# xkuubix/MonteCarlo-Gated-MIL

Measured on AMD Instinct MI355X. Metric: bags/sec × MCDO-samples (T=100) at N=2048,d=512; 1/2/4/8-GPU + %HBM roofline, higher is better.
Workload: dtype bf16

## Files before the change

montecarlo-gated-mil_amd/csrc/mcgmil_kernels.h:

```cpp
#pragma once
#include "mcgmil_device.h"

namespace mcgmil {

struct GateParams {
    const void* H;
    long long ldh;
    const int32_t* bag_off;
    int B, T, L, D, C, G, P;
    long long total_samples;
    const void* Wp;
    uint32_t wp_bytes;
    const float* bv;
    const float* bu;
    const float* wa;
    const float* ba;
    float sf, sa;
    uint32_t thr_f, thr_a;
    uint32_t thrx_f;
    uint32_t k0, k1;
    uint32_t bag_base;
    int t_base;
    const uint32_t* bag_ids;
    const int32_t* tile_bag;
// ... 59 lines not shown
            bag = (int)(R / per_bag);
            const long long local = R - (long long)bag * per_bag;
            t = (int)(local / Nb);
            n = (int)(local - (long long)t * Nb);
        }
        hrow = bag * Nb + n;
    } else if (R < p.total_samples) {
        if (p.tile_bag) {
            bag = p.tile_bag[R0 / BM];
            while ((long long)p.T * p.bag_off[bag + 1] <= R) ++bag;
        } else {
            bag = find_bag(p.bag_off, p.B, p.T, R);
        }
        const int ob = p.bag_off[bag];
        Nb = p.bag_off[bag + 1] - ob;
        const long long local = R - (long long)p.T * ob;
        if (narrow) {
            t = (int)((uint32_t)local / (uint32_t)Nb);
            n = (int)((uint32_t)local - (uint32_t)t * (uint32_t)Nb);
        } else {
            t = (int)(local / Nb);
            n = (int)(local - (long long)t * Nb);
        }
        hrow = ob + n;
    }
    int* ri = rinfo + kRowInfo * tid;
    ri[0] = hrow; ri[1] = t; ri[2] = n; ri[3] = bag; ri[4] = Nb;
    ri[5] = (int)(p.bag_ids ? p.bag_ids[bag] : p.bag_base + (uint32_t)bag);
}

#ifndef MCGMIL_KERNELS_TEMPLATES_ONLY
__global__ void plan_tiles_kernel(const int32_t* bag_off, int B, int T, long long total_samples,
                                  int BM, long long tiles, int32_t* tile_bag) {
    const long long i = (long long)blockIdx.x * blockDim.x + threadIdx.x;
    if (i >= tiles) return;
    const long long R = i * BM;
    tile_bag[i] = R < total_samples ? find_bag(bag_off, B, T, R) : 0;
}
#endif

__device__ __forceinline__ float gated_product_scaled(float ax, float by) {
    ax = fminf(fmaxf(ax, -43.280851226668903f), 43.280851226668903f);
    const float a = __builtin_amdgcn_exp2f(ax);
    const float b = __builtin_amdgcn_exp2f(by);
    const float ia = 1.0f + a;
    return (1.0f - a) * __builtin_amdgcn_rcpf(fmaf(ia, b, ia));
}

#ifndef MCGMIL_DIAG
#define MCGMIL_DIAG 0
#endif
#ifndef MCGMIL_PHILOX_ROUNDS
#define MCGMIL_PHILOX_ROUNDS 10
#endif

constexpr float kM2Log2e = -2.8853900817779268f;
constexpr float kMLog2e = -1.4426950408889634f;

struct HeadVec { f32x4 bv, bu, wa; };

template <int PPW>
__device__ __forceinline__ void load_head_vectors(const GateParams& p, int q0, int lane,
                                                  HeadVec (&hv)[PPW]) {
    const int DB = p.D >> 4;
#pragma unroll
    for (int jp = 0; jp < PPW; ++jp) {
        const int q = q0 + jp < p.P ? q0 + jp : p.P - 1;
        const int g = q / DB, db = q - g * DB;
        const int d0 = db * 16 + 4 * (lane >> 4);
        hv[jp].bv = *reinterpret_cast<const f32x4*>(p.bv + (size_t)g * p.D + d0) * kM2Log2e;
        hv[jp].bu = *reinterpret_cast<const f32x4*>(p.bu + (size_t)g * p.D + d0) * kMLog2e;
        hv[jp].wa = *reinterpret_cast<const f32x4*>(p.wa + (size_t)g * p.D + d0);
    }
}

struct Region {
    int bag, t0, t1, Nb, ob;
    int ntiles;
    long long S, rows;
};

constexpr int kFusedTiles = 32;
constexpr int kFusedHv = 256;
struct alignas(16) FusedConst {
    Region rg;
    uint32_t bagctr;
    int pad0;
    float ba[4];
    int cls[8];
    int pad1[8];
    int4 tile[kFusedTiles];
    float hv[3][kFusedHv];
};

#ifndef MCGMIL_FUSED_HV_LDS
#define MCGMIL_FUSED_HV_LDS 1
#endif
template <int PPW>
__device__ __forceinline__ void load_head_vectors_lds(const FusedConst* fc, int P, int q0, int lane,
                                                      HeadVec (&hv)[PPW]) {
#pragma unroll
    for (int jp = 0; jp < PPW; ++jp) {
        const int q = q0 + jp < P ? q0 + jp : P - 1;
        const int d = 16 * q + 4 * (lane >> 4);
        hv[jp].bv = *reinterpret_cast<const f32x4*>(fc->hv[0] + d);
        hv[jp].bu = *reinterpret_cast<const f32x4*>(fc->hv[1] + d);
        hv[jp].wa = *reinterpret_cast<const f32x4*>(fc->hv[2] + d);
    }
}

template <int RT, int PPW, int MAXC, bool ONE_CLASS, int RTV = RT>
__device__ __forceinline__ void fold_pairs(const GateParams& p, const f32x4 (&acc)[RT][2 * PPW],
                                           int q0, int lane, float (&part)[MAXC][RT],
                                           const HeadVec* pre = nullptr) {
    const int DB = p.D >> 4;
    const float av_s = p.sf * kM2Log2e, au_s = p.sf * kMLog2e;
#pragma unroll
    for (int jp = 0; jp < PPW; ++jp) {
        const int q = q0 + jp;
        if (q >= p.P) break;
        const int col = 16 * q + 4 * (lane >> 4);
        const int g = ONE_CLASS ? 0 : q / DB;
        const int d0 = col - g * p.D;
        f32x4 bvv, buv;
        f32x4 coef[MAXC];
        if (ONE_CLASS && pre) {
            bvv = pre[jp].bv;
            buv = pre[jp].bu;
            coef[0] = pre[jp].wa;
#pragma unroll
            for (int c = 1; c < MAXC; ++c) coef[c] = f32x4{0.f, 0.f, 0.f, 0.f};
        } else {
            bvv = *reinterpret_cast<const f32x4*>(p.bv + col);
            buv = *reinterpret_cast<const f32x4*>(p.bu + col);
            bvv *= kM2Log2e;
            buv *= kMLog2e;
#pragma unroll
            for (int c = 0; c < MAXC; ++c) {
                const int cc = ONE_CLASS ? g : c;
                const bool use = ONE_CLASS ? (c == 0) : ((c < p.C) && (p.G == 1 || c == g));
                const f32x4 w = *reinterpret_cast<const f32x4*>(p.wa + (size_t)(use ? cc : 0) * p.D + d0);
                coef[c] = use ? w : f32x4{0.f, 0.f, 0.f, 0.f};
            }
        }
#pragma unroll
        for (int rt = 0; rt < RTV; ++rt) {
#pragma unroll
            for (int v = 0; v < 4; ++v) {
                const float ax = fmaf(acc[rt][2 * jp][v], av_s, bvv[v]);
                const float by = fmaf(acc[rt][2 * jp + 1][v], au_s, buv[v]);
                if constexpr (ONE_CLASS) {
#if MCGMIL_DIAG & 8
                    part[0][rt] = fmaf(fmaf(ax, coef[0][v], by), ax, part[0][rt]);
                    continue;
#endif
                    const float a = __builtin_amdgcn_exp2f(fminf(fmaxf(ax, -43.280851226668903f),
                                                                 43.280851226668903f));
                    const float b = __builtin_amdgcn_exp2f(by);
                    const float ia = 1.0f + a;
                    const float r = __builtin_amdgcn_rcpf(fmaf(ia, b, ia));
                    part[0][rt] = fmaf(fmaf(-a, coef[0][v], coef[0][v]), r, part[0][rt]);
                } else {
                    const float pr = gated_product_scaled(ax, by);
#pragma unroll
                    for (int c = 0; c < MAXC; ++c) part[c][rt] = fmaf(pr, coef[c][v], part[c][rt]);
                }
            }
        }
    }
}

template <int BM, int MAXC>
__host__ __device__ constexpr int red_floats() { return kGateWaves * MAXC * 4 * BM; }

template <int BM, int MAXC, int ROWS = 16, bool AFFINE = false>
__device__ __forceinline__ void finish_scores(const GateParams& p, long long R0,
                                              float (&part)[MAXC][BM / ROWS], f32x4 zacc,
                                              bool zwave, float* red, float* zred,
                                              const int* rinfo, int one_class, int waves_per_gate,
                                              bool have_keep, bool keep, float* lg_out,
                                              float* z_out, long long obase,
                                              const FusedConst* fc = nullptr, int tile = 0) {
    constexpr int RT = BM / ROWS;
    constexpr int NG = 64 / ROWS;
    const int tid = threadIdx.x, lane = tid & 63, wave = tid >> 6;
    const int ncls = one_class < 0 ? MAXC : 1;
#pragma unroll
    for (int c = 0; c < MAXC; ++c) {
        if (c >= ncls) break;
        const int cls = one_class < 0 ? c : one_class;
        if (cls >= MAXC) break;
        float* dst = red + ((size_t)(wave * MAXC + cls) * NG + lane / ROWS) * BM + (lane % ROWS);
#pragma unroll
        for (int q = 0; q < RT; ++q) dst[ROWS * q] = part[c][q];
    }
    if (zwave && lane < 16) {
#pragma unroll
        for (int c = 0; c < MAXC; ++c) zred[c * BM + wave * 16 + lane] = zacc[c];
    }
    MCGMIL_STAMP(p, 5);
    __syncthreads();
    MCGMIL_STAMP(p, 6);
    const int r = wave * 16 + (lane & 15), c = lane >> 4;
    if (r >= BM || c >= p.C) return;
    int t, n, bag, Nb;
    uint32_t bagc;
    size_t orow;
    float bias;
    if constexpr (AFFINE) {
        const int4 tl = fc->tile[tile];
        t = tl.x, n = tl.y + r, bag = fc->rg.bag, Nb = fc->rg.Nb;
        bagc = fc->bagctr;
        orow = (size_t)(tl.z + r);
        bias = fc->ba[c];
    } else {
        const int* ri = rinfo + kRowInfo * r;
        if (ri[0] < 0) return;
        t = ri[1], n = ri[2], bag = ri[3], Nb = ri[4];
        bagc = (uint32_t)ri[5];
        orow = (size_t)(R0 + r - obase);
        bias = p.ba[c];
    }
    float s = 0.f;
    const int nw = waves_per_gate ? waves_per_gate : kGateWaves;
    for (int k = 0; k < nw; ++k) {
        const int w = waves_per_gate ? c * waves_per_gate + k : k;
        const float* src = red + (size_t)(w * MAXC + c) * NG * BM + r;
#pragma unroll
        for (int g = 0; g < NG; ++g) s += src[g * BM];
    }
    s += bias;
    if (p.keep_att) {
        const size_t abase = (size_t)p.T * p.C * (size_t)p.bag_off[bag];
        keep = p.keep_att[abase + ((size_t)t * p.C + c) * Nb + n] != 0;
    } else if (!have_keep) {
        keep = attention_keep(p.k0, p.k1, bagc, (uint32_t)(p.t_base + t), (uint32_t)c,
                              (uint32_t)n, p.thr_a);
    }
    const size_t o = orow * p.C + c;
    lg_out[o] = s * (keep ? p.sa : 0.f);
    z_out[o] = zred[c * BM + r] * p.sf;
}

constexpr int kSoftmaxRows = 16;

#ifndef MCGMIL_NT_A
#define MCGMIL_NT_A 1
#endif
__device__ __forceinline__ void store_a(float* dst, float v) {
#if MCGMIL_NT_A
    __builtin_nontemporal_store(v, dst);
#else
    *dst = v;
#endif
}

__device__ __forceinline__ void softmax_group(int ltid, bool active, int Nb, int C, const float* lg,
                                              const float* zz, float* Ao, float* Yo, float* sred) {
    const int tid = ltid, lane = ltid & 63, wave = ltid >> 6;
    if (Nb == 0) {
        if (active && tid < C) Yo[tid] = 0.f;
        return;
    }
    const int Nl = active ? Nb : 0;
    if (C == 2 && Nb <= 256 * kSoftmaxRows) {
        float (*sred2)[4] = reinterpret_cast<float (*)[4]>(sred);
        float e0[kSoftmaxRows], e1[kSoftmaxRows];
        float2 zr[kSoftmaxRows];
        float m0 = -INFINITY, m1 = -INFINITY;
#pragma unroll
        for (int k = 0; k < kSoftmaxRows; ++k) {
            const int n = tid + 256 * k;
            float2 l = make_float2(-INFINITY, -INFINITY);
            zr[k] = make_float2(0.f, 0.f);
            if (n < Nl) {
                l = *reinterpret_cast<const float2*>(lg + (size_t)n * 2);
                zr[k] = *reinterpret_cast<const float2*>(zz + (size_t)n * 2);
            }
            e0[k] = l.x;
            e1[k] = l.y;
            m0 = fmaxf(m0, e0[k]);
            m1 = fmaxf(m1, e1[k]);
        }
        m0 = wave_max(m0);
        m1 = wave_max(m1);
        if (lane == 0) { sred2[0][wave] = m0; sred2[1][wave] = m1; }
        __syncthreads();
        m0 = fmaxf(fmaxf(sred2[0][0], sred2[0][1]), fmaxf(sred2[0][2], sred2[0][3]));
        m1 = fmaxf(fmaxf(sred2[1][0], sred2[1][1]), fmaxf(sred2[1][2], sred2[1][3]));
        __syncthreads();
        float s0 = 0.f, y0 = 0.f, s1 = 0.f, y1 = 0.f;
#pragma unroll
        for (int k = 0; k < kSoftmaxRows; ++k) {
            const int n = tid + 256 * k;
            if (n < Nl) {
                const float2 z = zr[k];
                e0[k] = expf(e0[k] - m0);
                e1[k] = expf(e1[k] - m1);
                s0 += e0[k];
                s1 += e1[k];
                y0 = fmaf(e0[k], z.x, y0);
                y1 = fmaf(e1[k], z.y, y1);
            }
        }
        s0 = wave_sum(s0);
        y0 = wave_sum(y0);
        s1 = wave_sum(s1);
        y1 = wave_sum(y1);
        if (lane == 0) {
            sred2[0][wave] = s0; sred2[1][wave] = y0; sred2[2][wave] = s1; sred2[3][wave] = y1;
        }
        __syncthreads();
        s0 = (sred2[0][0] + sred2[0][1]) + (sred2[0][2] + sred2[0][3]);
        y0 = (sred2[1][0] + sred2[1][1]) + (sred2[1][2] + sred2[1][3]);
        s1 = (sred2[2][0] + sred2[2][1]) + (sred2[2][2] + sred2[2][3]);
        y1 = (sred2[3][0] + sred2[3][1]) + (sred2[3][2] + sred2[3][3]);
        __syncthreads();
// ... 52 lines not shown
                for (int k = 0; k < kSoftmaxRows; ++k) {
                    const int n = tid + 256 * k;
                    if (n < Nl) store_a(Aoc + n, e[k] * inv);
                }
            }
            if (active && tid == 0) Yo[c] = y * inv;
            continue;
        }
        float m = -INFINITY;
        for (int n = tid; n < Nl; n += 256) m = fmaxf(m, lg[(size_t)n * C + c]);
        m = wave_max(m);
        if (lane == 0) sr[0][wave] = m;
        __syncthreads();
        m = fmaxf(fmaxf(sr[0][0], sr[0][1]), fmaxf(sr[0][2], sr[0][3]));
        __syncthreads();
        float s = 0.f, y = 0.f;
        for (int n = tid; n < Nl; n += 256) {
            const size_t o = (size_t)n * C + c;
            const float e = expf(lg[o] - m);
            s += e;
            y = fmaf(e, zz[o], y);
        }
        s = wave_sum(s);
        y = wave_sum(y);
        if (lane == 0) { sr[0][wave] = s; sr[1][wave] = y; }
        __syncthreads();
        s = (sr[0][0] + sr[0][1]) + (sr[0][2] + sr[0][3]);
        y = (sr[1][0] + sr[1][1]) + (sr[1][2] + sr[1][3]);
        __syncthreads();
        const float inv = 1.0f / s;
        if (Ao) {
            float* Aoc = Ao + (size_t)c * Nb;
            for (int n = tid; n < Nl; n += 256) store_a(Aoc + n, expf(lg[(size_t)n * C + c] - m) * inv);
        }
        if (active && tid == 0) Yo[c] = y * inv;
    }
}

#ifndef MCGMIL_KERNELS_TEMPLATES_ONLY
__global__ __launch_bounds__(256) void softmax_pool_kernel(const int32_t* bag_off, int T, int C,
                                                           const float* logits, const float* zz,
                                                           float* Y, float* A) {
    __shared__ float sred[16];
    const int t = blockIdx.x, b = blockIdx.y;
    const int ob = bag_off[b];
    const int Nb = bag_off[b + 1] - ob;
    const size_t R0 = (size_t)T * ob + (size_t)t * Nb;
    softmax_group(threadIdx.x, true, Nb, C, logits + R0 * C, zz + R0 * C,
                  A ? A + (size_t)T * C * ob + (size_t)t * C * Nb : nullptr,
                  Y + ((size_t)b * T + t) * C, sred);
}
#endif

template <typename E> struct Raw;
template <> struct Raw<__bf16> { uint4 v; };
template <> struct Raw<float> { f32x4 lo, hi; };
__device__ __forceinline__ Raw<__bf16> load_raw(const __bf16* p) {
    Raw<__bf16> r; r.v = *reinterpret_cast<const uint4*>(p); return r;
}
__device__ __forceinline__ Raw<float> load_raw(const float* p) {
    Raw<float> r;
    r.lo = *reinterpret_cast<const f32x4*>(p);
    r.hi = *reinterpret_cast<const f32x4*>(p + 4);
    return r;
}
__device__ __forceinline__ void store_masked(const Raw<__bf16>& h, uint32_t kb, __bf16* dst) {
    uint4 v = h.v;
    v.x &= ((kb & 1u) ? 0x0000FFFFu : 0u) | ((kb & 2u) ? 0xFFFF0000u : 0u);
    v.y &= ((kb & 4u) ? 0x0000FFFFu : 0u) | ((kb & 8u) ? 0xFFFF0000u : 0u);
    v.z &= ((kb & 16u) ? 0x0000FFFFu : 0u) | ((kb & 32u) ? 0xFFFF0000u : 0u);
    v.w &= ((kb & 64u) ? 0x0000FFFFu : 0u) | ((kb & 128u) ? 0xFFFF0000u : 0u);
    *reinterpret_cast<uint4*>(dst) = v;
}
__device__ __forceinline__ void store_masked(const Raw<float>& h, uint32_t kb, float* dst) {
    f32x4 a = h.lo, b = h.hi;
    a.x = (kb & 1u) ? a.x : 0.f;   a.y = (kb & 2u) ? a.y : 0.f;
    a.z = (kb & 4u) ? a.z : 0.f;   a.w = (kb & 8u) ? a.w : 0.f;
    b.x = (kb & 16u) ? b.x : 0.f;  b.y = (kb & 32u) ? b.y : 0.f;
    b.z = (kb & 64u) ? b.z : 0.f;  b.w = (kb & 128u) ? b.w : 0.f;
    *reinterpret_cast<f32x4*>(dst) = a;
    *reinterpret_cast<f32x4*>(dst + 4) = b;
}

__device__ __forceinline__ void store_dropped(const Raw<__bf16>& h, uint4 o, uint32_t thrx,
                                              uint32_t inval, __bf16* dst) {
    uint4 v = h.v;
    v.x = __builtin_amdgcn_bitop3_b32(v.x, drop_mask16x2_flipped(o.x, thrx), inval, 0x10);
    v.y = __builtin_amdgcn_bitop3_b32(v.y, drop_mask16x2(o.y, thrx), inval, 0x10);
    v.z = __builtin_amdgcn_bitop3_b32(v.z, drop_mask16x2_flipped(o.z, thrx), inval, 0x10);
    v.w = __builtin_amdgcn_bitop3_b32(v.w, drop_mask16x2(o.w, thrx), inval, 0x10);
    *reinterpret_cast<uint4*>(dst) = v;
}
__device__ __forceinline__ uint32_t keep_lo(uint32_t m) { return ~(uint32_t)((int32_t)(m << 16) >> 16); }
__device__ __forceinline__ uint32_t keep_hi(uint32_t m) { return ~(uint32_t)((int32_t)m >> 16); }
__device__ __forceinline__ void store_dropped(const Raw<float>& h, uint4 o, uint32_t thrx,
                                              uint32_t inval, float* dst) {
    const uint32_t m0 = drop_mask16x2_flipped(o.x, thrx) | inval, m1 = drop_mask16x2(o.y, thrx) | inval;
    const uint32_t m2 = drop_mask16x2_flipped(o.z, thrx) | inval, m3 = drop_mask16x2(o.w, thrx) | inval;
    f32x4 a = h.lo, b = h.hi;
    a.x = __uint_as_float(__float_as_uint(a.x) & keep_lo(m0));
    a.y = __uint_as_float(__float_as_uint(a.y) & keep_hi(m0));
    a.z = __uint_as_float(__float_as_uint(a.z) & keep_lo(m1));
    a.w = __uint_as_float(__float_as_uint(a.w) & keep_hi(m1));
    b.x = __uint_as_float(__float_as_uint(b.x) & keep_lo(m2));
    b.y = __uint_as_float(__float_as_uint(b.y) & keep_hi(m2));
    b.z = __uint_as_float(__float_as_uint(b.z) & keep_lo(m3));
    b.w = __uint_as_float(__float_as_uint(b.w) & keep_hi(m3));
    *reinterpret_cast<f32x4*>(dst) = a;
    *reinterpret_cast<f32x4*>(dst + 4) = b;
}

constexpr int kPipeBM = 128;
#ifndef MCGMIL_VPM
#define MCGMIL_VPM 2
#endif
constexpr int VPM = MCGMIL_VPM;
#ifndef MCGMIL_SCHED
#define MCGMIL_SCHED 0
#endif
constexpr int HD = 2;
template <typename E>
__host__ __device__ constexpr int pipe_slots() { return 2; }

template <typename E, int MAXC>
__host__ __device__ constexpr size_t pipe_lds_bytes() {
    return (size_t)pipe_slots<E>() * kPipeBM * 32 * sizeof(E) + (size_t)red_floats<kPipeBM, MAXC>() * 4 +
           (size_t)MAXC * kPipeBM * 4 + (size_t)kRowInfo * kPipeBM * 4;
}

template <typename E>
__device__ __forceinline__ void load_classifier_lds(__amdgpu_buffer_rsrc_t wrs, uint32_t zsoff, int KS, E* zw) {
    for (int i = threadIdx.x; i < KS * 64; i += kGateThreads)
        *reinterpret_cast<f32x4*>(zw + (size_t)i * 8) = __builtin_bit_cast(
            f32x4, __builtin_amdgcn_raw_buffer_load_b128(wrs, (uint32_t)i * 8u * (uint32_t)sizeof(E), zsoff, 0));
}

template <typename E, int PPW, int MAXC, bool REPLAY, bool ONE_CLASS, bool EARLY_HV = true,
          bool ZL = false, bool ZLOAD = true, int RTV = kPipeBM / 16, bool AFFINE = false>
__device__ __forceinline__ void pipe_tile(const GateParams& p, long long R0, E* Xs, float* red,
                                          float* zred, const int* rinfo, float* lg_out,
                                          float* z_out, long long obase, E* zw = nullptr,
                                          const FusedConst* fc = nullptr, int tile = 0) {
    constexpr int BM = kPipeBM;
    constexpr int RT = BM / 16;
    constexpr int NJ = 2 * PPW;
    constexpr int SLOT = RT * 64 * 8;
    const int tid = threadIdx.x, lane = tid & 63, wave = tid >> 6;
    const int KS = p.L >> 5;

    int hrow;
    uint32_t cn, ct, cb;
    if constexpr (AFFINE) {
        static_assert(!REPLAY, "the affine rows have no replay masks");
        const int4 tl = fc->tile[tile];
        cn = (uint32_t)(tl.y + wave * 16 + (lane & 15));
        hrow = fc->rg.ob + (int)cn;
        ct = (uint32_t)(p.t_base + tl.x);
        cb = fc->bagctr;
    } else {
        const int* ri = rinfo + kRowInfo * (wave * 16 + (lane & 15));
        hrow = ri[0];
        cn = (uint32_t)ri[2], ct = (uint32_t)(p.t_base + ri[1]), cb = (uint32_t)ri[5];
    }
    const bool valid = AFFINE || hrow >= 0;
    const int kq = lane >> 4;
    const E* hsrc = reinterpret_cast<const E*>(p.H) + (size_t)(valid ? hrow : 0) * p.ldh + kq * 8;
    const uint8_t* kfe = REPLAY ? p.keep_feat + (size_t)(valid ? R0 + wave * 16 + (lane & 15) : 0) *
                                                    (p.L >> 3) + kq
                                : nullptr;

    const uint32_t inval = valid ? 0u : 0xFFFFFFFFu;
    auto stage = [&](int s, const Raw<E>& h, E* slot) {
        if constexpr (REPLAY) {
            const uint32_t kb = kfe[(size_t)(s < KS ? s : KS - 1) * 4];
            store_masked(h, kb & ~inval, slot + tid * 8);
        } else {
#if MCGMIL_DIAG & 4
            const uint4 o = make_uint4(cn * 0x9E3779B9u + (uint32_t)s, ct ^ cb, cn + ct, (uint32_t)s * 77u);
#else
            const uint4 o = philox4x32_10<true, MCGMIL_PHILOX_ROUNDS>((uint32_t)(s * 4 + kq), cn, ct, cb, p.k0, p.k1);
#endif
            store_dropped(h, o, p.thrx_f, inval, slot + tid * 8);
        }
    };

    const __amdgpu_buffer_rsrc_t wrs = make_rsrc(p.Wp, p.wp_bytes);
    const uint32_t tile_bytes = (uint32_t)KS * 512u * (uint32_t)sizeof(E);
    constexpr uint32_t kStepBytes = 512u * (uint32_t)sizeof(E);
    const int q0 = __builtin_amdgcn_readfirstlane(wave) * PPW;
    uint32_t wsoff[NJ];
#pragma unroll
    for (int j = 0; j < NJ; ++j) {
        int q = q0 + (j >> 1);
        q = q < p.P ? q : p.P - 1;
        wsoff[j] = (uint32_t)(2 * q + (j & 1)) * tile_bytes;
    }
    const uint32_t zsoff = (uint32_t)(2 * p.P) * tile_bytes;
    const uint32_t lane_b = (uint32_t)lane * 8u * (uint32_t)sizeof(E);
    auto wfrag = [&](uint32_t soff) { return load_frag_buf<E>(wrs, lane_b, soff); };

    f32x4 acc[RT][NJ];
#pragma unroll
    for (int rt = 0; rt < RT; ++rt)
#pragma unroll
        for (int j = 0; j < NJ; ++j) acc[rt][j] = f32x4{0.f, 0.f, 0.f, 0.f};
    f32x4 zacc = {0.f, 0.f, 0.f, 0.f};

    auto kstep = [&](int s, const E* cur, E* nxt, const Frag<E> (&w)[NJ], const Frag<E>& z,
                     Frag<E> (&wn)[NJ], Frag<E>& zn, const Raw<E>& h, Raw<E>& hn) {
        const int s1 = s + 1 < KS ? s + 1 : KS - 1;
        const int sh = s + HD < KS ? s + HD : KS - 1;
#if MCGMIL_DIAG & 2
#pragma unroll
        for (int j = 0; j < NJ; ++j) wn[j] = w[j];
        zn = z;
#else
#pragma unroll
        for (int j = 0; j < NJ; ++j) wn[j] = wfrag(wsoff[j] + (uint32_t)s1 * kStepBytes);
        if constexpr (!ZL) zn = wfrag(zsoff + (uint32_t)s1 * kStepBytes);
#endif
#if MCGMIL_DIAG & 1
        hn = h;
#else
        if (RTV == RT || wave < RTV) hn = load_raw(hsrc + (size_t)sh * 32);
#endif
#pragma unroll
        for (int rt = 0; rt < RTV; ++rt) {
            const Frag<E> x = load_frag(cur + (size_t)(rt * 64 + lane) * 8);
#pragma unroll
            for (int j = 0; j < NJ; ++j) acc[rt][j] = mma(w[j], x, acc[rt][j]);
        }
        const Frag<E> xz = load_frag(cur + (size_t)tid * 8);
        if constexpr (ZL) zacc = mma(load_frag(zw + (size_t)(s * 64 + lane) * 8), xz, zacc);
        else zacc = mma(z, xz, zacc);
        if (RTV == RT || wave < RTV) stage(s + 1, h, nxt);
        if constexpr (sizeof(E) == 2 && PPW == 2) {
#if MCGMIL_SCHED == 1
            __builtin_amdgcn_sched_group_barrier(0x020, NJ + 2, 0);
            __builtin_amdgcn_sched_group_barrier(0x100, 3, 0);
#pragma unroll
            for (int rt = 0; rt < RT; ++rt) {
#pragma unroll
                for (int j = 0; j < NJ; ++j) {
                    __builtin_amdgcn_sched_group_barrier(0x008, 1, 0);
                    __builtin_amdgcn_sched_group_barrier(0x002, VPM, 0);
                }
                if (rt + 2 < RT) __builtin_amdgcn_sched_group_barrier(0x100, 1, 0);
            }
            __builtin_amdgcn_sched_group_barrier(0x008, 1, 0);
            __builtin_amdgcn_sched_group_barrier(0x002, VPM, 0);
#else
#pragma unroll
            for (int i = 0; i < RTV * NJ + 1; ++i) {
                __builtin_amdgcn_sched_group_barrier(0x008, 1, 0);
                __builtin_amdgcn_sched_group_barrier(0x002, VPM, 0);
            }
#endif
        }
#if MCGMIL_DIAG & 128
        asm volatile("s_waitcnt lgkmcnt(0)" ::: "memory");
#else
        __syncthreads();
#endif
    };

    constexpr bool kEarlyHV = EARLY_HV && ONE_CLASS && sizeof(E) == 2;
    HeadVec hvec[PPW];
    {
        Frag<E> wA[NJ], wB[NJ], zA, zB;
        Raw<E> hA{}, hB{};
        if (RTV == RT || wave < RTV) {
            hA = load_raw(hsrc);
            hB = load_raw(hsrc + 32);
        }
#pragma unroll
        for (int j = 0; j < NJ; ++j) wA[j] = wfrag(wsoff[j]);
        if constexpr (ZL) {
            if constexpr (ZLOAD) load_classifier_lds<E>(wrs, zsoff, KS, zw);
        } else {
            zA = wfrag(zsoff);
        }
        if (RTV == RT || wave < RTV) stage(0, hA, Xs);
        __syncthreads();
        MCGMIL_STAMP(p, 2);

        if constexpr (kEarlyHV) load_head_vectors<PPW>(p, q0, lane, hvec);
        kstep(0, Xs, Xs + SLOT, wA, zA, wB, zB, hB, hA);
        kstep(1, Xs + SLOT, Xs, wB, zB, wA, zA, hA, hB);
#if MCGMIL_DIAG & 16
        if (KS > 1000)
#endif
        for (int s = 2; s < KS; s += 2) {
            kstep(s, Xs, Xs + SLOT, wA, zA, wB, zB, hB, hA);
            kstep(s + 1, Xs + SLOT, Xs, wB, zB, wA, zA, hA, hB);
        }
    }
    MCGMIL_STAMP(p, 3);

    float part[MAXC][RT];
#pragma unroll
    for (int c = 0; c < MAXC; ++c)
#pragma unroll
        for (int rt = 0; rt < RT; ++rt) part[c][rt] = 0.f;
    constexpr bool kLdsHV = MCGMIL_FUSED_HV_LDS && AFFINE && ONE_CLASS && !kEarlyHV;
    if constexpr (kLdsHV) load_head_vectors_lds<PPW>(fc, p.P, q0, lane, hvec);
    fold_pairs<RT, PPW, MAXC, ONE_CLASS, RTV>(p, acc, q0, lane, part, kEarlyHV || kLdsHV ? hvec : nullptr);
    MCGMIL_STAMP(p, 4);
    int one_class = -1;
    if constexpr (ONE_CLASS && AFFINE) one_class = __builtin_amdgcn_readfirstlane(fc->cls[wave]);
    else if constexpr (ONE_CLASS) one_class = q0 < p.P ? q0 / (p.D >> 4) : MAXC;
    finish_scores<BM, MAXC, 16, AFFINE>(p, R0, part, zacc, true, red, zred, rinfo, one_class,
                                        ONE_CLASS ? (p.D >> 4) / PPW : 0, false, true, lg_out, z_out,
                                        obase, fc, tile);
    MCGMIL_STAMP(p, 7);
}

#ifndef MCGMIL_XCD_TILES
#define MCGMIL_XCD_TILES 1
#endif
__device__ __forceinline__ long long xcd_tile(unsigned b, unsigned n, int bags) {
#if MCGMIL_XCD_TILES
    const unsigned x = b & 7u, q = n >> 3, r = n & 7u;
    const unsigned l = (x < r ? x * (q + 1) : r * (q + 1) + (x - r) * q) + (b >> 3);
    return (long long)(bags >= 8 ? l : b);
#else
    (void)n;
    (void)bags;
    return (long long)b;
#endif
}

template <typename E, int PPW, int MAXC, bool REPLAY, bool ONE_CLASS, bool PROBE = false, int RTV = kPipeBM / 16>
__global__ __launch_bounds__(kGateThreads) void gate_pipe_kernel(const GateParams p) {
    extern __shared__ __attribute__((aligned(16))) unsigned char smem[];
    constexpr int BM = kPipeBM;
    E* Xs = reinterpret_cast<E*>(smem);
    float* red = reinterpret_cast<float*>(smem + (size_t)pipe_slots<E>() * BM * 32 * sizeof(E));
    float* zred = red + red_floats<BM, MAXC>();
    int* rinfo = reinterpret_cast<int*>(zred + MAXC * BM);
    const long long R0 = RTV == BM / 16 ? xcd_tile(blockIdx.x, gridDim.x, p.B) * BM
                                        : p.tile_row0 + (long long)blockIdx.x * (16 * RTV);

    if constexpr (PROBE) clock_probe(p, 0);
    MCGMIL_STAMP(p, 0);
    fill_row_table<BM, 16 * RTV>(p, R0, rinfo);
    __syncthreads();
    MCGMIL_STAMP(p, 1);
    pipe_tile<E, PPW, MAXC, REPLAY, ONE_CLASS, true, false, true, RTV>(p, R0, Xs, red, zred, rinfo, p.logits,
                                                                       p.zz, 0);
    if constexpr (PROBE) clock_probe(p, 1);
}

#ifndef MCGMIL_FUSED_XCD
#define MCGMIL_FUSED_XCD 1
#endif
#ifndef MCGMIL_FUSED_EARLY_HV
#define MCGMIL_FUSED_EARLY_HV 0
#endif
#ifndef MCGMIL_FUSED_NMAJOR
#define MCGMIL_FUSED_NMAJOR 1
#endif
#ifndef MCGMIL_FUSED_CAP
#define MCGMIL_FUSED_CAP 4096
#endif
template <int MAXC>
__host__ __device__ constexpr int fused_cap() { return MAXC <= 2 ? MCGMIL_FUSED_CAP : MCGMIL_FUSED_CAP / 4; }

template <typename E, int MAXC>
__host__ __device__ constexpr size_t fused_lds_bytes() {
    return pipe_lds_bytes<E, MAXC>() + (size_t)kRowInfo * kPipeBM * 4
           + (size_t)2 * fused_cap<MAXC>() * MAXC * 4
           + (size_t)2 * 16 * 4 + sizeof(FusedConst);
}
static_assert(kFusedTiles * kPipeBM >= MCGMIL_FUSED_CAP, "FusedConst::tile holds a whole region");

__host__ __device__ inline bool fused_affine(int uniform_rows, int cap) {
    return uniform_rows > 0 && uniform_rows % kPipeBM == 0 && uniform_rows <= cap;
}

#ifndef MCGMIL_FUSED_ZL
#define MCGMIL_FUSED_ZL 1
#endif
template <typename E>
__host__ __device__ constexpr bool fused_zl() { return MCGMIL_FUSED_ZL && sizeof(E) == 2; }
template <typename E, int MAXC>
__host__ __device__ constexpr size_t fused_kernel_lds_bytes(int L) {
    return fused_lds_bytes<E, MAXC>() + (fused_zl<E>() ? (size_t)(L / 32) * 512 * sizeof(E) : 0);
}

__host__ __device__ inline int region_t_groups(int Nb, int T, int cap) {
    if (Nb <= 0) return T;
    if (Nb > cap) return 1;
    const int ts = cap / Nb;
    return ts < T ? ts : T;
}

__device__ __forceinline__ int region_tile(const Region& rg, int i) {
#if MCGMIL_FUSED_NMAJOR
    const int G = rg.t1 - rg.t0;
    if (G > 1 && rg.Nb % kPipeBM == 0) return (i % G) * (rg.Nb / kPipeBM) + i / G;
#endif
    return i;
}

__device__ __forceinline__ GateParams reload_kernarg_params(const GateParams& p) {
#if __HIP_DEVICE_COMPILE__
    typedef __attribute__((address_space(4))) const GateParams* KernargParams;
    KernargParams q = (KernargParams)__builtin_amdgcn_kernarg_segment_ptr();
    asm volatile("" : "+s"(q));
    return *q;
#else
    return p;
#endif
}

__device__ __forceinline__ bool decode_region(const GateParams& p, int g, int cap, Region& rg) {
    int b, j, ts;
    if (p.uniform_rows > 0) {
        ts = p.region_t;
        const int rpb = (p.T + ts - 1) / ts;
        if (MCGMIL_FUSED_XCD && (p.B & 7) == 0) {
            const int k = g >> 3;
            b = 8 * (k / rpb) + (g & 7);
            j = k - (k / rpb) * rpb;
        } else {
            b = g / rpb;
            j = g - b * rpb;
        }
        if (b >= p.B) return false;
    } else {
        if (g >= p.region_off[p.B]) return false;
        b = find_bag(p.region_off, p.B, 1, g);
        j = g - p.region_off[b];
        ts = region_t_groups(p.bag_off[b + 1] - p.bag_off[b], p.T, cap);
    }
    rg.bag = b;
    rg.ob = p.bag_off[b];
    rg.Nb = p.bag_off[b + 1] - rg.ob;
    rg.t0 = j * ts;
    rg.t1 = rg.t0 + ts < p.T ? rg.t0 + ts : p.T;
    rg.S = (long long)p.T * rg.ob + (long long)rg.t0 * rg.Nb;
    rg.rows = (long long)(rg.t1 - rg.t0) * rg.Nb;
    rg.ntiles = (int)((rg.rows + kPipeBM - 1) / kPipeBM);
    return true;
}

template <int BM>
__device__ __forceinline__ void fill_row_table_region(const GateParams& p, const Region& rg,
                                                      long long R0, int* rinfo) {
    const int tid = threadIdx.x;
    if (tid >= BM) return;
    const long long rho = R0 + tid - rg.S;
    int hrow = -1, t = 0, n = 0;
    if (rho < rg.rows) {
        const uint32_t r = (uint32_t)rho;
        const uint32_t tt = r / (uint32_t)rg.Nb;
        n = (int)(r - tt * (uint32_t)rg.Nb);
        t = rg.t0 + (int)tt;
        hrow = rg.ob + n;
    }
    int* ri = rinfo + kRowInfo * tid;
    ri[0] = hrow; ri[1] = t; ri[2] = n; ri[3] = rg.bag; ri[4] = rg.Nb;
    ri[5] = (int)(p.bag_ids ? p.bag_ids[rg.bag] : p.bag_base + (uint32_t)rg.bag);
}


template <int PPW, int MAXC, bool ONE_CLASS>
__device__ __forceinline__ void fill_fused_const(const GateParams& p, const Region& rg, FusedConst* fc) {
    const int tid = threadIdx.x;
    if (tid == 0) {
        fc->rg = rg;
        fc->bagctr = p.bag_ids ? p.bag_ids[rg.bag] : p.bag_base + (uint32_t)rg.bag;
    }
    if (tid < MAXC) fc->ba[tid] = tid < p.C ? p.ba[tid] : 0.f;
    if (tid < kGateWaves) {
        const int q0 = tid * PPW, DB = p.D >> 4;
        int g = 0;
        while ((g + 1) * DB <= q0) ++g;
        fc->cls[tid] = ONE_CLASS && q0 < p.P ? g : MAXC;
    }
    if (tid < rg.ntiles && tid < kFusedTiles) {
        const int G = rg.t1 - rg.t0, nbt = rg.Nb / kPipeBM;
        const int dv = MCGMIL_FUSED_NMAJOR ? G : nbt;
        int qt = 0;
        while ((qt + 1) * dv <= tid) ++qt;
        const int rem = tid - qt * dv;
        const int tg = MCGMIL_FUSED_NMAJOR ? rem : qt, nb = MCGMIL_FUSED_NMAJOR ? qt : rem;
        fc->tile[tid] = make_int4(rg.t0 + tg, nb * kPipeBM, tg * rg.Nb + nb * kPipeBM, 0);
    }
    if (ONE_CLASS && tid < 16 * p.P && tid < kFusedHv) {
        fc->hv[0][tid] = p.bv[tid] * kM2Log2e;
        fc->hv[1][tid] = p.bu[tid] * kMLog2e;
        fc->hv[2][tid] = p.wa[tid];
    }
}

template <typename E, int PPW, int MAXC, bool ONE_CLASS, bool PROBE, bool AFFINE>
__device__ __forceinline__ void fused_region(const GateParams& p) {
    extern __shared__ __attribute__((aligned(16))) unsigned char smem[];
    constexpr int BM = kPipeBM;
    constexpr int CAP = fused_cap<MAXC>();
    E* Xs = reinterpret_cast<E*>(smem);
    float* red = reinterpret_cast<float*>(smem + (size_t)pipe_slots<E>() * BM * 32 * sizeof(E));
    float* zred = red + red_floats<BM, MAXC>();
    int* rinfo = reinterpret_cast<int*>(zred + MAXC * BM);
    float* slg = reinterpret_cast<float*>(rinfo + 2 * kRowInfo * BM);
    float* szz = slg + CAP * MAXC;
    float* sred = szz + CAP * MAXC;
    FusedConst* fc = reinterpret_cast<FusedConst*>(sred + 32);

#if MCGMIL_DIAG & 64
    {
        const long long R0 = (long long)blockIdx.x * BM;
        fill_row_table<BM>(p, R0, rinfo);
        __syncthreads();
        pipe_tile<E, PPW, MAXC, false, ONE_CLASS>(p, R0, Xs, red, zred, rinfo, p.logits, p.zz, 0);
        return;
    }
#endif
    Region rg;
    if (!decode_region(p, (int)blockIdx.x, CAP, rg)) return;
    if constexpr (PROBE) clock_probe(p, 0);
    const int ntiles = (int)((rg.rows + BM - 1) / BM);
    Region* srg = &fc->rg;
    if constexpr (AFFINE) fill_fused_const<PPW, MAXC, ONE_CLASS>(p, rg, fc);
    else if (threadIdx.x == 0) *srg = rg;
    __syncthreads();
    E* zw = reinterpret_cast<E*>(smem + fused_lds_bytes<E, MAXC>());
    if constexpr (fused_zl<E>())
        load_classifier_lds<E>(make_rsrc(p.Wp, p.wp_bytes), (uint32_t)(2 * p.P) * (uint32_t)(p.L >> 5) * 512u *
                                   (uint32_t)sizeof(E), p.L >> 5, zw);
    for (int i = 0; i < ntiles; ++i) {
        const GateParams pt = reload_kernarg_params(p);
        if constexpr (AFFINE) {
            MCGMIL_STAMP(pt, 0);
            MCGMIL_STAMP(pt, 1);
            pipe_tile<E, PPW, MAXC, false, ONE_CLASS, MCGMIL_FUSED_EARLY_HV, fused_zl<E>(), false, BM / 16, true>(
                pt, 0, Xs, red, zred, nullptr, slg, szz, 0, zw, fc, i);
        } else {
            Region* qr = srg;
            asm volatile("" : "+v"(qr));
            int* ri = rinfo + (i & 1) * kRowInfo * BM;
            MCGMIL_STAMP(pt, 0);
            {
                const Region r = *qr;
                fill_row_table_region<BM>(pt, r, r.S + (long long)region_tile(r, i) * BM, ri);
            }
            __syncthreads();
            MCGMIL_STAMP(pt, 1);
            const Region r = *qr;
            const bool lds = r.Nb <= CAP;
            pipe_tile<E, PPW, MAXC, false, ONE_CLASS, MCGMIL_FUSED_EARLY_HV, fused_zl<E>(), false>(
                pt, r.S + (long long)region_tile(r, i) * BM, Xs, red, zred, ri, lds ? slg : pt.logits,
                lds ? szz : pt.zz, lds ? r.S : 0, zw);
        }
    }
    __syncthreads();
#if MCGMIL_DIAG & 32
    if (ntiles >= 0) return;
#endif
    rg = *srg;
    const bool in_lds = AFFINE || rg.Nb <= CAP;

    const int G = rg.t1 - rg.t0;
    const int half = threadIdx.x >> 8, ltid = threadIdx.x & 255;
    for (int j0 = 0; j0 < G; j0 += 2) {
        const bool act = j0 + half < G;
        const int j = act ? j0 + half : j0;
        const long long row0 = (long long)j * rg.Nb;
        const float* lgj = in_lds ? slg + row0 * p.C : p.logits + (rg.S + row0) * p.C;
        const float* zzj = in_lds ? szz + row0 * p.C : p.zz + (rg.S + row0) * p.C;
        float* Ao = p.A ? p.A + (size_t)p.T * p.C * rg.ob + (size_t)(rg.t0 + j) * p.C * rg.Nb : nullptr;
// ... 293 lines not shown
```

Before: 969,800.

## Reuse each wave's own staged X fragment in registers and rotate LDS row-tile order

The staging step now returns the dropout-masked H fragment it writes to LDS, so each wave keeps its own row tile in registers. That fragment is used directly for the first MMA group and for the classifier MMA, which removes one or two LDS fragment loads per k-step. Row tiles are then visited in a per-wave rotated order, so different waves start on different LDS regions, and the rotation is undone when partial scores are written to the reduction buffer. This costs some extra registers and changes the scheduling-barrier counts, which could hurt occupancy or instruction interleaving.

```diff
diff --git a/montecarlo-gated-mil_amd/csrc/mcgmil_kernels.h b/montecarlo-gated-mil_amd/csrc/mcgmil_kernels.h
--- a/montecarlo-gated-mil_amd/csrc/mcgmil_kernels.h
+++ b/montecarlo-gated-mil_amd/csrc/mcgmil_kernels.h
@@ -256,7 +256,7 @@
 template <int BM, int MAXC>
 __host__ __device__ constexpr int red_floats() { return kGateWaves * MAXC * 4 * BM; }
 
-template <int BM, int MAXC, int ROWS = 16, bool AFFINE = false>
+template <int BM, int MAXC, int ROWS = 16, bool AFFINE = false, bool ROT = false>
 __device__ __forceinline__ void finish_scores(const GateParams& p, long long R0,
                                               float (&part)[MAXC][BM / ROWS], f32x4 zacc,
                                               bool zwave, float* red, float* zred,
@@ -275,7 +275,7 @@
         if (cls >= MAXC) break;
         float* dst = red + ((size_t)(wave * MAXC + cls) * NG + lane / ROWS) * BM + (lane % ROWS);
 #pragma unroll
-        for (int q = 0; q < RT; ++q) dst[ROWS * q] = part[c][q];
+        for (int q = 0; q < RT; ++q) dst[ROWS * (ROT ? (wave + q) & (RT - 1) : q)] = part[c][q];
     }
     if (zwave && lane < 16) {
 #pragma unroll
@@ -534,14 +534,15 @@
     *reinterpret_cast<f32x4*>(dst + 4) = b;
 }
 
-__device__ __forceinline__ void store_dropped(const Raw<__bf16>& h, uint4 o, uint32_t thrx,
-                                              uint32_t inval, __bf16* dst) {
+__device__ __forceinline__ uint4 store_dropped(const Raw<__bf16>& h, uint4 o, uint32_t thrx,
+                                               uint32_t inval, __bf16* dst) {
     uint4 v = h.v;
     v.x = __builtin_amdgcn_bitop3_b32(v.x, drop_mask16x2_flipped(o.x, thrx), inval, 0x10);
     v.y = __builtin_amdgcn_bitop3_b32(v.y, drop_mask16x2(o.y, thrx), inval, 0x10);
     v.z = __builtin_amdgcn_bitop3_b32(v.z, drop_mask16x2_flipped(o.z, thrx), inval, 0x10);
     v.w = __builtin_amdgcn_bitop3_b32(v.w, drop_mask16x2(o.w, thrx), inval, 0x10);
     *reinterpret_cast<uint4*>(dst) = v;
+    return v;
 }
 __device__ __forceinline__ uint32_t keep_lo(uint32_t m) { return ~(uint32_t)((int32_t)(m << 16) >> 16); }
 __device__ __forceinline__ uint32_t keep_hi(uint32_t m) { return ~(uint32_t)((int32_t)m >> 16); }
@@ -570,6 +571,15 @@
 #ifndef MCGMIL_SCHED
 #define MCGMIL_SCHED 0
 #endif
+#ifndef MCGMIL_OWN_FRAG
+#define MCGMIL_OWN_FRAG 1
+#endif
+#ifndef MCGMIL_OWN_ROT
+#define MCGMIL_OWN_ROT 1
+#endif
+#ifndef MCGMIL_OWN_ORDER
+#define MCGMIL_OWN_ORDER 0
+#endif
 constexpr int HD = 2;
 template <typename E>
 __host__ __device__ constexpr int pipe_slots() { return 2; }
@@ -621,25 +631,34 @@
                                                     (p.L >> 3) + kq
                                 : nullptr;
 
+    constexpr bool OWN = MCGMIL_OWN_FRAG && !REPLAY && sizeof(E) == 2 && RTV == RT;
+    constexpr bool ROT = OWN && MCGMIL_OWN_ROT;
     const uint32_t inval = valid ? 0u : 0xFFFFFFFFu;
-    auto stage = [&](int s, const Raw<E>& h, E* slot) {
+    auto stage = [&](int s, const Raw<E>& h, E* slot) -> Frag<E> {
         if constexpr (REPLAY) {
             const uint32_t kb = kfe[(size_t)(s < KS ? s : KS - 1) * 4];
             store_masked(h, kb & ~inval, slot + tid * 8);
+            return Frag<E>{};
         } else {
 #if MCGMIL_DIAG & 4
             const uint4 o = make_uint4(cn * 0x9E3779B9u + (uint32_t)s, ct ^ cb, cn + ct, (uint32_t)s * 77u);
 #else
             const uint4 o = philox4x32_10<true, MCGMIL_PHILOX_ROUNDS>((uint32_t)(s * 4 + kq), cn, ct, cb, p.k0, p.k1);
 #endif
-            store_dropped(h, o, p.thrx_f, inval, slot + tid * 8);
+            if constexpr (OWN) {
+                return __builtin_bit_cast(Frag<E>, store_dropped(h, o, p.thrx_f, inval, slot + tid * 8));
+            } else {
+                store_dropped(h, o, p.thrx_f, inval, slot + tid * 8);
+                return Frag<E>{};
+            }
         }
     };
 
     const __amdgpu_buffer_rsrc_t wrs = make_rsrc(p.Wp, p.wp_bytes);
     const uint32_t tile_bytes = (uint32_t)KS * 512u * (uint32_t)sizeof(E);
     constexpr uint32_t kStepBytes = 512u * (uint32_t)sizeof(E);
-    const int q0 = __builtin_amdgcn_readfirstlane(wave) * PPW;
+    const int wave_u = __builtin_amdgcn_readfirstlane(wave);
+    const int q0 = wave_u * PPW;
     uint32_t wsoff[NJ];
 #pragma unroll
     for (int j = 0; j < NJ; ++j) {
@@ -659,7 +678,8 @@
     f32x4 zacc = {0.f, 0.f, 0.f, 0.f};
 
     auto kstep = [&](int s, const E* cur, E* nxt, const Frag<E> (&w)[NJ], const Frag<E>& z,
-                     Frag<E> (&wn)[NJ], Frag<E>& zn, const Raw<E>& h, Raw<E>& hn) {
+                     Frag<E> (&wn)[NJ], Frag<E>& zn, const Raw<E>& h, Raw<E>& hn,
+                     const Frag<E>& xo, Frag<E>& xn) {
         const int s1 = s + 1 < KS ? s + 1 : KS - 1;
         const int sh = s + HD < KS ? s + HD : KS - 1;
 #if MCGMIL_DIAG & 2
@@ -676,20 +696,37 @@
 #else
         if (RTV == RT || wave < RTV) hn = load_raw(hsrc + (size_t)sh * 32);
 #endif
-#pragma unroll
-        for (int rt = 0; rt < RTV; ++rt) {
-            const Frag<E> x = load_frag(cur + (size_t)(rt * 64 + lane) * 8);
-#pragma unroll
-            for (int j = 0; j < NJ; ++j) acc[rt][j] = mma(w[j], x, acc[rt][j]);
-        }
-        const Frag<E> xz = load_frag(cur + (size_t)tid * 8);
-        if constexpr (ZL) zacc = mma(load_frag(zw + (size_t)(s * 64 + lane) * 8), xz, zacc);
-        else zacc = mma(z, xz, zacc);
-        if (RTV == RT || wave < RTV) stage(s + 1, h, nxt);
+        auto zmma = [&](const Frag<E>& xz) {
+            if constexpr (ZL) zacc = mma(load_frag(zw + (size_t)(s * 64 + lane) * 8), xz, zacc);
+            else zacc = mma(z, xz, zacc);
+        };
+        if constexpr (ROT) {
+#pragma unroll
+            for (int j = 0; j < NJ; ++j) acc[0][j] = mma(w[j], xo, acc[0][j]);
+            zmma(xo);
+#pragma unroll
+            for (int i = 1; i < RT; ++i) {
+                const uint32_t ro = (uint32_t)((wave_u + i) & (RT - 1)) * (uint32_t)(64 * 8 * sizeof(E));
+                const Frag<E> x = load_frag(reinterpret_cast<const E*>(
+                    reinterpret_cast<const unsigned char*>(cur + (size_t)lane * 8) + ro));
+#pragma unroll
+                for (int j = 0; j < NJ; ++j) acc[i][j] = mma(w[j], x, acc[i][j]);
+            }
+        } else {
+#pragma unroll
+            for (int rt = 0; rt < RTV; ++rt) {
+                const Frag<E> x = load_frag(cur + (size_t)(rt * 64 + lane) * 8);
+#pragma unroll
+                for (int j = 0; j < NJ; ++j) acc[rt][j] = mma(w[j], x, acc[rt][j]);
+            }
+            if constexpr (OWN) zmma(xo);
+            else zmma(load_frag(cur + (size_t)tid * 8));
+        }
+        if (RTV == RT || wave < RTV) xn = stage(s + 1, h, nxt);
         if constexpr (sizeof(E) == 2 && PPW == 2) {
 #if MCGMIL_SCHED == 1
             __builtin_amdgcn_sched_group_barrier(0x020, NJ + 2, 0);
-            __builtin_amdgcn_sched_group_barrier(0x100, 3, 0);
+            __builtin_amdgcn_sched_group_barrier(0x100, OWN ? 2 : 3, 0);
 #pragma unroll
             for (int rt = 0; rt < RT; ++rt) {
 #pragma unroll
@@ -697,10 +734,18 @@
                     __builtin_amdgcn_sched_group_barrier(0x008, 1, 0);
                     __builtin_amdgcn_sched_group_barrier(0x002, VPM, 0);
                 }
-                if (rt + 2 < RT) __builtin_amdgcn_sched_group_barrier(0x100, 1, 0);
+                if (rt + (ROT ? 3 : 2) < RT) __builtin_amdgcn_sched_group_barrier(0x100, 1, 0);
             }
             __builtin_amdgcn_sched_group_barrier(0x008, 1, 0);
             __builtin_amdgcn_sched_group_barrier(0x002, VPM, 0);
+#elif MCGMIL_OWN_ORDER == 1
+            if constexpr (ROT) __builtin_amdgcn_sched_group_barrier(0x100, ZL ? 3 : 2, 0);
+#pragma unroll
+            for (int i = 0; i < RTV * NJ + 1; ++i) {
+                __builtin_amdgcn_sched_group_barrier(0x008, 1, 0);
+                __builtin_amdgcn_sched_group_barrier(0x002, VPM, 0);
+                if (ROT && i % NJ == NJ - 1 && i / NJ < RT - 3) __builtin_amdgcn_sched_group_barrier(0x100, 1, 0);
+            }
 #else
 #pragma unroll
             for (int i = 0; i < RTV * NJ + 1; ++i) {
@@ -732,19 +777,20 @@
         } else {
             zA = wfrag(zsoff);
         }
-        if (RTV == RT || wave < RTV) stage(0, hA, Xs);
+        Frag<E> xA{}, xB{};
+        if (RTV == RT || wave < RTV) xA = stage(0, hA, Xs);
         __syncthreads();
         MCGMIL_STAMP(p, 2);
 
         if constexpr (kEarlyHV) load_head_vectors<PPW>(p, q0, lane, hvec);
-        kstep(0, Xs, Xs + SLOT, wA, zA, wB, zB, hB, hA);
-        kstep(1, Xs + SLOT, Xs, wB, zB, wA, zA, hA, hB);
+        kstep(0, Xs, Xs + SLOT, wA, zA, wB, zB, hB, hA, xA, xB);
+        kstep(1, Xs + SLOT, Xs, wB, zB, wA, zA, hA, hB, xB, xA);
 #if MCGMIL_DIAG & 16
         if (KS > 1000)
 #endif
         for (int s = 2; s < KS; s += 2) {
-            kstep(s, Xs, Xs + SLOT, wA, zA, wB, zB, hB, hA);
-            kstep(s + 1, Xs + SLOT, Xs, wB, zB, wA, zA, hA, hB);
+            kstep(s, Xs, Xs + SLOT, wA, zA, wB, zB, hB, hA, xA, xB);
+            kstep(s + 1, Xs + SLOT, Xs, wB, zB, wA, zA, hA, hB, xB, xA);
         }
     }
     MCGMIL_STAMP(p, 3);
@@ -761,7 +807,7 @@
     int one_class = -1;
     if constexpr (ONE_CLASS && AFFINE) one_class = __builtin_amdgcn_readfirstlane(fc->cls[wave]);
     else if constexpr (ONE_CLASS) one_class = q0 < p.P ? q0 / (p.D >> 4) : MAXC;
-    finish_scores<BM, MAXC, 16, AFFINE>(p, R0, part, zacc, true, red, zred, rinfo, one_class,
+    finish_scores<BM, MAXC, 16, AFFINE, ROT>(p, R0, part, zacc, true, red, zred, rinfo, one_class,
                                         ONE_CLASS ? (p.D >> 4) / PPW : 0, false, true, lg_out, z_out,
                                         obase, fc, tile);
     MCGMIL_STAMP(p, 7);
```

Result: no change. 973,800 (median of 6 runs) (+0.4%).

## Precompute attention dropout keep bits into LDS and unroll score reduction

Applied to the files above, without the earlier changes.

In the fused affine path, attention-dropout keep masks are generated once per region as packed bytes in LDS, with 16 threads per tile each running Philox for 8 rows. finish_scores then reads a single bit instead of recomputing the RNG per row and class. The partial-sum reduction over waves is fully unrolled with all loads issued up front, and the score phase is remapped so all lanes are used, with rows taken as tid mod BM. It costs extra LDS, a serial per-class loop in the fill step, and relies on keep_byte matching attention_keep's bits exactly.

```diff
diff --git a/montecarlo-gated-mil_amd/csrc/mcgmil_kernels.h b/montecarlo-gated-mil_amd/csrc/mcgmil_kernels.h
--- a/montecarlo-gated-mil_amd/csrc/mcgmil_kernels.h
+++ b/montecarlo-gated-mil_amd/csrc/mcgmil_kernels.h
@@ -165,6 +165,18 @@
 
 constexpr int kFusedTiles = 32;
 constexpr int kFusedHv = 256;
+#ifndef MCGMIL_FUSED_KEEP_LDS
+#define MCGMIL_FUSED_KEEP_LDS 1
+#endif
+#ifndef MCGMIL_SCORE_UNROLL
+#define MCGMIL_SCORE_UNROLL 1
+#endif
+#ifndef MCGMIL_SCORE_FULL_LANES
+#define MCGMIL_SCORE_FULL_LANES 1
+#endif
+#ifndef MCGMIL_SCORE_LATE_INDEX
+#define MCGMIL_SCORE_LATE_INDEX 1
+#endif
 struct alignas(16) FusedConst {
     Region rg;
     uint32_t bagctr;
@@ -256,6 +268,25 @@
 template <int BM, int MAXC>
 __host__ __device__ constexpr int red_floats() { return kGateWaves * MAXC * 4 * BM; }
 
+template <int NW, int WSTRIDE, int NG, int GSTRIDE>
+__device__ __forceinline__ float sum_partials(const float* src, int nw) {
+    float v[NW * NG];
+#pragma unroll
+    for (int k = 0; k < NW; ++k)
+#pragma unroll
+        for (int g = 0; g < NG; ++g) v[k * NG + g] = src[(k < nw ? k : 0) * WSTRIDE + g * GSTRIDE];
+    float s = 0.f;
+#pragma unroll
+    for (int k = 0; k < NW; ++k)
+#pragma unroll
+        for (int g = 0; g < NG; ++g) s = k < nw ? s + v[k * NG + g] : s;
+    return s;
+}
+
+__device__ __forceinline__ const uint8_t* fused_keep_bits(const FusedConst* fc) {
+    return reinterpret_cast<const uint8_t*>(fc + 1);
+}
+
 template <int BM, int MAXC, int ROWS = 16, bool AFFINE = false>
 __device__ __forceinline__ void finish_scores(const GateParams& p, long long R0,
                                               float (&part)[MAXC][BM / ROWS], f32x4 zacc,
@@ -284,18 +315,28 @@
     MCGMIL_STAMP(p, 5);
     __syncthreads();
     MCGMIL_STAMP(p, 6);
-    const int r = wave * 16 + (lane & 15), c = lane >> 4;
+    constexpr bool kFullLanes = MCGMIL_SCORE_FULL_LANES && AFFINE && (BM & (BM - 1)) == 0;
+    int stid = tid;
+#if MCGMIL_SCORE_LATE_INDEX
+    if constexpr (AFFINE) asm volatile("" : "+v"(stid));
+#endif
+    const int r = kFullLanes ? (stid & (BM - 1)) : (stid >> 6) * 16 + (stid & 15);
+    const int c = kFullLanes ? (int)((unsigned)stid / (unsigned)BM) : (stid & 63) >> 4;
     if (r >= BM || c >= p.C) return;
     int t, n, bag, Nb;
     uint32_t bagc;
     size_t orow;
     float bias;
+    [[maybe_unused]] uint32_t kbits = 0;
     if constexpr (AFFINE) {
         const int4 tl = fc->tile[tile];
         t = tl.x, n = tl.y + r, bag = fc->rg.bag, Nb = fc->rg.Nb;
         bagc = fc->bagctr;
         orow = (size_t)(tl.z + r);
         bias = fc->ba[c];
+#if MCGMIL_FUSED_KEEP_LDS
+        if (!p.keep_att) kbits = fused_keep_bits(fc)[(uint32_t)((tl.z + r) >> 3) * (uint32_t)p.C + (uint32_t)c];
+#endif
     } else {
         const int* ri = rinfo + kRowInfo * r;
         if (ri[0] < 0) return;
@@ -306,16 +347,23 @@
     }
     float s = 0.f;
     const int nw = waves_per_gate ? waves_per_gate : kGateWaves;
+    const float* src0 = red + (size_t)((waves_per_gate ? c * waves_per_gate : 0) * MAXC + c) * NG * BM + r;
+#if MCGMIL_SCORE_UNROLL
+    if (nw == 4) s = sum_partials<4, MAXC * NG * BM, NG, BM>(src0, 4);
+    else s = sum_partials<kGateWaves, MAXC * NG * BM, NG, BM>(src0, nw);
+#else
     for (int k = 0; k < nw; ++k) {
-        const int w = waves_per_gate ? c * waves_per_gate + k : k;
-        const float* src = red + (size_t)(w * MAXC + c) * NG * BM + r;
+        const float* src = src0 + (size_t)k * MAXC * NG * BM;
 #pragma unroll
         for (int g = 0; g < NG; ++g) s += src[g * BM];
     }
+#endif
     s += bias;
     if (p.keep_att) {
         const size_t abase = (size_t)p.T * p.C * (size_t)p.bag_off[bag];
         keep = p.keep_att[abase + ((size_t)t * p.C + c) * Nb + n] != 0;
+    } else if (AFFINE && MCGMIL_FUSED_KEEP_LDS) {
+        keep = (kbits >> (n & 7)) & 1u;
     } else if (!have_keep) {
         keep = attention_keep(p.k0, p.k1, bagc, (uint32_t)(p.t_base + t), (uint32_t)c,
                               (uint32_t)n, p.thr_a);
@@ -818,12 +866,20 @@
 template <int MAXC>
 __host__ __device__ constexpr int fused_cap() { return MAXC <= 2 ? MCGMIL_FUSED_CAP : MCGMIL_FUSED_CAP / 4; }
 
+template <int MAXC>
+__host__ __device__ constexpr size_t fused_keep_bytes() {
+    return MCGMIL_FUSED_KEEP_LDS ? (size_t)fused_cap<MAXC>() * MAXC / 8 : 0;
+}
+
 template <typename E, int MAXC>
 __host__ __device__ constexpr size_t fused_lds_bytes() {
     return pipe_lds_bytes<E, MAXC>() + (size_t)kRowInfo * kPipeBM * 4
            + (size_t)2 * fused_cap<MAXC>() * MAXC * 4
-           + (size_t)2 * 16 * 4 + sizeof(FusedConst);
-}
+           + (size_t)2 * 16 * 4 + sizeof(FusedConst)
+           + fused_keep_bytes<MAXC>();
+}
+static_assert(sizeof(FusedConst) % 16 == 0 && fused_keep_bytes<2>() % 16 == 0 && fused_keep_bytes<4>() % 16 == 0,
+              "the classifier fragments after them stay 16-byte aligned");
 static_assert(kFusedTiles * kPipeBM >= MCGMIL_FUSED_CAP, "FusedConst::tile holds a whole region");
 
 __host__ __device__ inline bool fused_affine(int uniform_rows, int cap) {
@@ -920,9 +976,19 @@
 template <int PPW, int MAXC, bool ONE_CLASS>
 __device__ __forceinline__ void fill_fused_const(const GateParams& p, const Region& rg, FusedConst* fc) {
     const int tid = threadIdx.x;
+    const uint32_t bagctr = p.bag_ids ? p.bag_ids[rg.bag] : p.bag_base + (uint32_t)rg.bag;
+    auto tile_of = [&](int i) {
+        const int G = rg.t1 - rg.t0, nbt = rg.Nb / kPipeBM;
+        const int dv = MCGMIL_FUSED_NMAJOR ? G : nbt;
+        int qt = 0;
+        while ((qt + 1) * dv <= i) ++qt;
+        const int rem = i - qt * dv;
+        const int tg = MCGMIL_FUSED_NMAJOR ? rem : qt, nb = MCGMIL_FUSED_NMAJOR ? qt : rem;
+        return make_int4(rg.t0 + tg, nb * kPipeBM, tg * rg.Nb + nb * kPipeBM, 0);
+    };
     if (tid == 0) {
         fc->rg = rg;
-        fc->bagctr = p.bag_ids ? p.bag_ids[rg.bag] : p.bag_base + (uint32_t)rg.bag;
+        fc->bagctr = bagctr;
     }
     if (tid < MAXC) fc->ba[tid] = tid < p.C ? p.ba[tid] : 0.f;
     if (tid < kGateWaves) {
@@ -931,15 +997,18 @@
         while ((g + 1) * DB <= q0) ++g;
         fc->cls[tid] = ONE_CLASS && q0 < p.P ? g : MAXC;
     }
-    if (tid < rg.ntiles && tid < kFusedTiles) {
-        const int G = rg.t1 - rg.t0, nbt = rg.Nb / kPipeBM;
-        const int dv = MCGMIL_FUSED_NMAJOR ? G : nbt;
-        int qt = 0;
-        while ((qt + 1) * dv <= tid) ++qt;
-        const int rem = tid - qt * dv;
-        const int tg = MCGMIL_FUSED_NMAJOR ? rem : qt, nb = MCGMIL_FUSED_NMAJOR ? qt : rem;
-        fc->tile[tid] = make_int4(rg.t0 + tg, nb * kPipeBM, tg * rg.Nb + nb * kPipeBM, 0);
-    }
+    if (tid < rg.ntiles && tid < kFusedTiles) fc->tile[tid] = tile_of(tid);
+#if MCGMIL_FUSED_KEEP_LDS
+    if (!p.keep_att && tid < 16 * rg.ntiles && tid < 16 * kFusedTiles) {
+        const int4 tl = tile_of(tid >> 4);
+        const uint32_t blk = (uint32_t)(tid & 15);
+        uint8_t* kb = const_cast<uint8_t*>(fused_keep_bits(fc)) + (((uint32_t)tl.z >> 3) + blk) * (uint32_t)p.C;
+        for (int c = 0; c < p.C; ++c)
+            kb[c] = (uint8_t)keep_byte(philox4x32_10(((uint32_t)tl.y >> 3) + blk, (uint32_t)c,
+                                                     (uint32_t)(p.t_base + tl.x) | 0x80000000u, bagctr,
+                                                     p.k0, p.k1), p.thr_a);
+    }
+#endif
     if (ONE_CLASS && tid < 16 * p.P && tid < kFusedHv) {
         fc->hv[0][tid] = p.bv[tid] * kM2Log2e;
         fc->hv[1][tid] = p.bu[tid] * kMLog2e;
```

New measurement: 956,800 before, 968,000 after (median of 6 runs). 1.01x the previous value.
